# TinyMPC/tinympc-matlab

Measured on AMD Instinct MI355X. Metric: ADMM iterations/s, batched quadrotor nx=12 nu=4 N=50 (instance-iterations/s, whole job), higher is better.
Workload: dtype f64

## Files before the change

### __graft_entry__.py

```python
from __future__ import annotations

import hashlib
import importlib.util
import os
import shutil
import subprocess
import sys

ROOT = os.path.dirname(os.path.abspath(__file__))
if ROOT not in sys.path:
    sys.path.insert(0, ROOT)
PKG_DIR = os.path.join(ROOT, "tinympc-matlab_amd")
PKG_NAME = "tinympc_matlab_amd"
CSRC = os.path.join(PKG_DIR, "csrc")
HIP_LIB = os.path.join(PKG_DIR, "libtinympc_hip.so")
ORACLE_DIR = os.path.join(ROOT, "oracle")
REFERENCE_SRC = "/root/reference/src/codegen_src"

HIP_SOURCES = ["tinympc_kernels.hip", "tinympc_precompute_rows.hip", "tinympc_solve.hip", "tinympc_solve_b.hip", "tinympc_solve_fam.hip", "tinympc_solve_adapt.hip", "tinympc_imod_a.hip", "tinympc_solve_c.hip", "tinympc_solve_d.hip", "tinympc_solve_dr.hip", "tinympc_lean_d.hip", "tinympc_solve_dw.hip", "tinympc_solve_dx.hip", "tinympc_jit.hip", "tinympc_solve_m.hip", "tinympc_precompute_large.hip", "tinympc_handle.hip", "tinympc_plan.hip", "tinympc_session.hip", "tinympc_capi.hip",
               "tinympc_codegen.hip"]
HIP_LINTED = ["tinympc_precompute_rows.hip", "tinympc_solve.hip", "tinympc_solve_b.hip", "tinympc_solve_fam.hip", "tinympc_solve_adapt.hip", "tinympc_imod_a.hip",
              "tinympc_solve_c.hip", "tinympc_solve_d.hip", "tinympc_solve_dr.hip", "tinympc_lean_d.hip", "tinympc_solve_dw.hip", "tinympc_solve_dx.hip"]
JIT_EMBEDDED = ["tinympc_device.h", "tinympc_sweep.h", "tinympc_fam_red.h", "tinympc_solve_d_chain.h", "tinympc_solve_dw_chain.h", "tinympc_solve_dx_chain.h",
                "tinympc_solve_e_common.h", "tinympc_solve_dwide.h", "tinympc_solve_d.hip", "tinympc_solve_dw.hip", "tinympc_solve_dx.hip", "tinympc_solve_e.hip",
                "tinympc_solve_f.hip"]
_ROCKET = ["-DTINY_JIT_NX=6", "-DTINY_JIT_NU=3", "-DTINY_JIT_N=100", "-DTINY_JIT_CT=0", "-DTINY_JIT_FAM=1"]
_ROCKET_FAM = ["-DTINY_JIT_E_NROUND=1", "-DTINY_JIT_E_NCONE=2", "-DTINY_JIT_E_CONES={0,0,2},{0,6,8}", "-DTINY_JIT_E_NLX=1", "-DTINY_JIT_E_NLU=0"]
HIP_BUILTINS = [
    ("k_builtin_e_rocket100", "tinympc_solve_e.hip",
     _ROCKET + ["-DTINY_JIT_E_WPG=8", "-DTINY_JIT_E_WPS=2", "-DTINY_JIT_E_S=13"] + _ROCKET_FAM +
     ["-DTINY_JIT_E_GC_LDS=0", "-DTINY_JIT_E_GL_LDS=0", "-DTINY_JIT_E_LX_LDS=0", "-DTINY_JIT_E_KFAM=1", "-DTINY_JIT_E_DREG=1"]),
    ("k_builtin_f_rocket100", "tinympc_solve_f.hip", _ROCKET + ["-DTINY_JIT_F_WPG=4", "-DTINY_JIT_F_S=7"] + _ROCKET_FAM + ["-DTINY_JIT_F_KFAM=1"]),
    ("k_builtin_f_rocket100_session", "tinympc_solve_f.hip", _ROCKET + ["-DTINY_JIT_F_WPG=4", "-DTINY_JIT_F_S=7"] + _ROCKET_FAM + ["-DTINY_JIT_F_KFAM=1", "-DTINY_JIT_F_SESSION=1"]),
]
_NO_FAM = ["-DTINY_JIT_E_NROUND=0", "-DTINY_JIT_E_NCONE=0", "-DTINY_JIT_E_CONES={-1,0,0}", "-DTINY_JIT_E_NLX=0", "-DTINY_JIT_E_NLU=0"]
for _name, _nx, _nu, _N, _wpg, _S in (("cartpole20", 4, 1, 20, 2, 3), ("quadrotor50", 12, 4, 50, 4, 4)):
    for _suffix, _ct, _extra in (("", 1, []), ("_var", 0, []), ("_session", 0, ["-DTINY_JIT_F_SESSION=1"])):
# ... 44 lines not shown
        f.write(digest)


def _run(cmd, **kw):
    print("+", " ".join(cmd), flush=True)
    subprocess.run(cmd, check=True, **kw)


def device_asm_path(source: str) -> str:
    return os.path.join(BUILD_DIR, os.path.splitext(source)[0] + "-hip-amdgcn-amd-amdhsa-gfx950.s")


def _compile_one(hipcc: str, source: str, headers, force: bool) -> str:
    src = os.path.join(CSRC, source)
    obj = os.path.join(BUILD_DIR, os.path.splitext(source)[0] + ".o")
    digest = _hash([src] + headers, HIP_CFLAGS)
    if force or not _up_to_date(obj, digest):
        _run([hipcc] + HIP_CFLAGS + ["-save-temps=obj", "-c", src, "-o", obj])
        _stamp(obj, digest)
    return obj


def write_embedded_sources() -> str:
    os.makedirs(BUILD_DIR, exist_ok=True)
    out = os.path.join(BUILD_DIR, "tinympc_jit_embedded.inc")
    parts = ["// generated by __graft_entry__.write_embedded_sources() from tinympc-matlab_amd/csrc -- do not edit\n"]
    for i, name in enumerate(JIT_EMBEDDED):
        with open(os.path.join(CSRC, name)) as f:
            text = f.read()
        assert ')TINYSRC"' not in text
        pieces, cur = [], ""
# ... 233 lines not shown
```

### tinympc-matlab_amd/csrc/tinympc_device.h

```cpp
#pragma once
#ifndef __HIPCC_RTC__
#include <hip/hip_runtime.h>
#endif

namespace tinympc {

__host__ __device__ inline size_t ops_doubles(int W, int KT) { return (size_t)2 * W * KT + 3 * W; }

__host__ __device__ inline size_t table_rows(int N) { return (size_t)N + 2; }

constexpr int V_PAD = 4;
__host__ __device__ inline size_t v_rows(int N) { return (size_t)N + 1 + 2 * V_PAD; }
__host__ __device__ inline size_t tables_doubles(int W, int N) { return 3 * table_rows(N) * W + W; }

#if defined(__HIPCC__) || defined(__HIPCC_RTC__)
__device__ __forceinline__ void host_store(double *p, double v) { __hip_atomic_store(p, v, __ATOMIC_RELAXED, __HIP_MEMORY_SCOPE_SYSTEM); }
#endif

struct PrecomputeParams {
    int nx, nu;
    double rho;
    const double *A, *B, *fdyn, *Qd, *Rd;
    double *Kinf, *Pinf, *Quu_inv, *AmBKt, *APf, *BPf;
    int *info;
// ... 266 lines not shown
hipError_t launch_build_operators(const OperatorParams &p, hipStream_t stream);
hipError_t launch_build_tables(const TableParams &p, hipStream_t stream);
hipError_t launch_store_inst_refs(const InstRefStoreParams &p, hipStream_t stream);
hipError_t launch_build_inst_tables(const InstTableParams &p, hipStream_t stream);
hipError_t launch_fill_inst_models(const InstModelFillParams &p, hipStream_t stream);
hipError_t launch_store_inst_diag(const InstDiagParams &p, hipStream_t stream);
enum class SolveExt { Box, Families, Adaptive, InstRefs, InstBounds, InstModels };
hipError_t launch_solve_a(const SolveParams &p, SolveExt ext, int W, int KT, size_t lds_bytes, hipStream_t stream);
hipError_t launch_solve_b(const SolveParams &p, int W, int KT, size_t lds_bytes, hipStream_t stream);
size_t solve_b_lds_bytes(int nx, int nu, int N, int W);
constexpr int WAVES_PER_GROUP_B = 4;
bool solve_d_supported(int nx, int nu, int N, bool const_tables);
hipError_t launch_solve_d(const SolveParams &p, hipStream_t stream);
hipError_t launch_solve_d_refill(const SolveParams &p, hipStream_t stream);
hipError_t launch_solve_d_lean(const SolveParams &p, hipStream_t stream);
int solve_d_workgroups(int nu, int N, bool const_tables, int groups);
size_t solve_d_lds_bytes(int nu, int N, bool const_tables);
int solve_d_resident_workgroups(int wpg);
int solve_d_wavefronts_per_workgroup(int nu, int N, bool const_tables);
bool solve_dw_supported(int nx, int nu, int N, bool const_tables);
hipError_t launch_solve_dw(const SolveParams &p, hipStream_t stream);
int solve_dw_workgroups(int nu, int N, int groups);
size_t solve_dw_lds_bytes(int nu, int N);
bool solve_dx_supported(int nx, int nu, int N, bool const_tables);
hipError_t launch_solve_dx(const SolveParams &p, hipStream_t stream);
int solve_dx_workgroups(int nu, int N, int groups);
size_t solve_dx_lds_bytes(int nu, int N);
hipError_t launch_solve_c(const SolveParams &p, int W, int KT, size_t lds_bytes, hipStream_t stream);
hipError_t launch_build_chunk_tables(const ChunkTableParams &p, hipStream_t stream);
size_t f_input_table_doubles(int nu, int S);
// ... 50 lines not shown
```

### tinympc-matlab_amd/csrc/tinympc_plan.hip

```cpp
#include <cstring>
#include "tinympc_handle.h"

using namespace tinympc;
using namespace tinympc::host;

namespace {

void arm_completion_flag(tinympc_solver *s, SolveParams &p) {
    if (!p.host_sol) return;
    s->session_seq += 1;
    p.host_seq = (double)s->session_seq;
    s->flag_pending = true;
}

void decide_layout_d_variants(tinympc_solver *s) {
    if (!s->layout_d) return;
    if (s->d_varying < 0 && !s->tables_const()) {
        if (s->W == 16 && !s->d_jit && solve_d_supported(s->nx, s->nu, s->N, false)) {
            s->d_varying = 1;
        } else {
            s->d_varying_jit = solve_jit_supported(s->W, s->nx, s->nu, s->N, false);
            s->d_varying = s->d_varying_jit ? 1 : 0;
        }
    }
// ... 215 lines not shown
    return !jit || solve_jit_refill_supported(s->W, s->nx, s->nu, s->N, ct);
}

static bool lean_applies(const tinympc_solver *s, const LaunchPlan &pl) {
    if (pl.kernel != KernelId::D_COMPILED || s->W != 16 || pl.adaptive || pl.families || s->zero_copy_tick || s->st.max_iter <= 0)
        return false;
    if (pl.inst_models) return false;
    if (refill_applies(s, pl)) return false;
    const char *env = getenv("TINYMPC_LEAN");
    const int mode = env ? atoi(env) : -1;
    if (mode == 0) return false;
    if (mode == 1) return true;
    const bool reachable = s->st.abs_pri_tol > 0.0 && s->st.abs_dua_tol > 0.0;
    return s->st.check_termination != 1 || !reachable;
}

int launch(tinympc_solver *s, bool timed) {
    int rc;
    s->flag_pending = false;
    if ((rc = resolve_plan(s))) return rc;
    const LaunchPlan pl = current_plan(s);
    const bool fam = pl.families, adaptive = pl.adaptive;
    if (s->inst_tables() && !pl.inst_refs) {
        const bool r = s->inst.refs(), b = s->inst.bounds, m = s->inst.models;
        const char *what[3], *back[3];
        int n = 0;
        if (r) { what[n] = "per-instance references (set_x_ref_batch / set_u_ref_batch)"; back[n++] = "tinympc_set_x_ref / tinympc_set_u_ref return to shared references"; }
        if (b) { what[n] = "per-instance bounds (set_bound_constraints_batch)"; back[n++] = "tinympc_set_bound_constraints returns to shared bounds"; }
        if (m) { what[n] = "per-instance models (set_model_batch)"; back[n++] = "tinympc_clear_model_batch returns to the shared model"; }
        std::string subj, way;
// ... 88 lines not shown
    if (refill_applies(s, pl) && !p.x0_mirror && !p.u0_host && !p.host_sol) {
        if (!s->drefill && (rc = dalloc(s, &s->drefill, 1))) return rc;
        HIP_TRY(hipMemsetAsync(s->drefill, 0, sizeof(int), s->stream));
        p.refill_next = s->drefill;
    }
    if (timed) HIP_TRY(hipEventRecord(s->ev0, s->stream));
    switch (pl.kernel) {
        case KernelId::M:
            p.ctab = s->dctab;
            HIP_TRY(launch_solve_m(p, s->stream));
            break;
        case KernelId::D_JIT:
            HIP_TRY(launch_solve_jit(p, s->W, s->stream, pl.inst_models));
            break;
        case KernelId::D_COMPILED:
            if (lean_applies(s, pl) && !p.x0_mirror && !p.u0_host && !p.refill_next) HIP_TRY(launch_solve_d_lean(p, s->stream));
            else HIP_TRY(s->W == 64 ? launch_solve_dx(p, s->stream) : s->W == 32 ? launch_solve_dw(p, s->stream) : launch_solve_d(p, s->stream));
            break;
        case KernelId::E:
            p.ctab = s->dctab_e; p.chunk_len = s->e_chunk_len; p.chunk_count = s->e_wpg; p.chunk_levels = 1;
            HIP_TRY(launch_solve_e(p, s->fs, s->stream));
            break;
        case KernelId::F:
            p.ctab = s->dctab_f; p.ftab = s->dftab; p.chunk_len = s->f_chunk_len; p.chunk_count = s->f_chunks; p.chunk_levels = 4;
            arm_completion_flag(s, p);
            HIP_TRY(launch_solve_f(p, s->f_fs, s->stream));
            break;
        case KernelId::C:
            p.ctab = s->dctab; p.chunk_len = s->chunk_len; p.chunk_count = s->chunk_count; p.chunk_levels = s->chunk_levels;
            arm_completion_flag(s, p);
            HIP_TRY(launch_solve_c(p, s->W, s->KT, s->lds_bytes_c, s->stream));
// ... 57 lines not shown
    if (pl.inst_refs) {
        const std::string w = std::string(s->inst.refs() ? " per-instance-refs" : "") + (s->inst.bounds ? " per-instance-bounds" : "") +
                              (pl.inst_models ? " per-instance-models" : "");
        const char *words = w.c_str();
        if (pl.kernel == KernelId::D_JIT) {
            if ((rc = bind_device(s))) return rc;
            solve_jit_describe(s->W, s->nx, s->nu, s->N, true, false, false, buf, (size_t)len, true, pl.inst_models);
            strncat(buf, words, (size_t)len - strlen(buf) - 1);
            strncat(buf, " goal", (size_t)len - strlen(buf) - 1);
        } else if (pl.inst_models && models_want_d(s) && s->inst.d_models == 0) {
            if ((rc = bind_device(s))) return rc;
            solve_jit_describe(s->W, s->nx, s->nu, s->N, true, false, false, buf, (size_t)len, false, true);
            strncat(buf, words, (size_t)len - strlen(buf) - 1);
        } else {
            snprintf(buf, (size_t)len, "compiled-in layout=%c%s%s%s", pl.layout, words, pl.kernel == KernelId::D_COMPILED ? " goal" : "",
                     lean_applies(s, pl) ? " lean" : "");
        }
        return TINYMPC_OK;
    }
    if (!pl.adaptive && !s->f_sig.empty() && !s->f_ok && pl.kernel != KernelId::E && pl.kernel != KernelId::D_JIT && pl.kernel != KernelId::D_COMPILED)
        solve_f_describe(s->nx, s->nu, s->N, ct, pl.families, s->f_fs, buf, (size_t)len);
    else if (!pl.adaptive && !s->e_sig.empty() && !s->e_ok && pl.kernel != KernelId::F && pl.kernel != KernelId::D_JIT && pl.kernel != KernelId::D_COMPILED)
        solve_e_describe(s->nx, s->nu, s->N, ct, pl.families, s->fs, buf, (size_t)len);
    else if (pl.kernel == KernelId::F) solve_f_describe(s->nx, s->nu, s->N, ct, pl.families, s->f_fs, buf, (size_t)len);
    else if (pl.kernel == KernelId::E) solve_e_describe(s->nx, s->nu, s->N, ct, pl.families, s->fs, buf, (size_t)len);
    else if (pl.kernel == KernelId::D_JIT || (s->d_jit_asked && !s->layout_d && !s->layout_m)) {
        if ((rc = bind_device(s))) return rc;
        solve_jit_describe(s->W, s->nx, s->nu, s->N, ct, pl.families && !pl.adaptive, pl.adaptive && !pl.families, buf, (size_t)len);
        if (pl.kernel == KernelId::D_JIT && refill_applies(s, pl)) strncat(buf, " slot-refill", (size_t)len - strlen(buf) - 1);
    } else snprintf(buf, (size_t)len, "compiled-in layout=%c%s%s", pl.layout, refill_applies(s, pl) ? " slot-refill" : "", lean_applies(s, pl) ? " lean" : "");
    return TINYMPC_OK;
}

}
```

### tinympc-matlab_amd/csrc/tinympc_solve_d.hip

```cpp
#if defined(TINY_BUILTIN) && !defined(TINY_JIT)
#define TINY_JIT 1
#endif
#ifndef TINY_JIT
#include <atomic>
#endif
#include <type_traits>

#include "tinympc_device.h"
#include "tinympc_sweep.h"

#ifndef TINY_REFILL
#if defined(TINY_JIT_REFILL) && TINY_JIT_REFILL
#define TINY_REFILL 1
#else
#define TINY_REFILL 0
#endif
#endif

#ifndef TINY_LEAN
#define TINY_LEAN 0
#endif
#if TINY_LEAN && (TINY_REFILL || defined(TINY_JIT))
#error "TINY_LEAN: compiled-in plain kernels only"
#endif

#define TINY_STR2(x) #x
#define TINY_STR(x) TINY_STR2(x)
namespace tinympc {
template <int NX, int NU>
struct DStep;
}

#ifdef TINY_JIT
#define D_NX TINY_JIT_NX
#define D_NU TINY_JIT_NU
#include "tinympc_solve_d_chain.h"
#else
#define D_NX 12
// ... 3 lines not shown
#define D_NU 1
#include "tinympc_solve_d_chain.h"
#endif

namespace tinympc {

template <int I, int E, class F>
__device__ __forceinline__ void static_for(F &&f) {
    if constexpr (I < E) {
        f(std::integral_constant<int, I>{});
        static_for<I + 1, E>(f);
    }
}

constexpr int D_OPS_DOUBLES = 2 * 16 * 16;
#ifdef TINY_D_GROUP
constexpr int D_GROUP = TINY_D_GROUP;
constexpr int D_FIRST = TINY_D_FIRST;
#else
#if TINY_REFILL
constexpr int D_GROUP = 12;
constexpr int D_FIRST = 4;
#else
constexpr int D_GROUP = 23;
constexpr int D_FIRST = 4;
#endif
#endif
#ifdef TINY_JIT_VREG
constexpr int D_VREG_MAX = TINY_JIT_VREG;
#else
constexpr int D_VREG_MAX = 24;
#endif
constexpr int D_LDS_PER_CU = 160 * 1024;
__host__ __device__ constexpr int d_d_doubles(int nu, int N) { return ((N - 1) * 4 * nu + 1) & ~1; }
__host__ __device__ constexpr int d_tab_doubles(int N) { return 3 * (N + 2) * 16 + 16; }
constexpr int D_FAM_DOUBLES = 3 * MAX_LIN_ROWS * 16;
constexpr int D_ADAPT_DOUBLES = 5 * 16 * 16;
constexpr int D_IMOD_STRIDE = D_OPS_DOUBLES + 16;
constexpr int D_IMOD_WAVE_DOUBLES = 4 * D_IMOD_STRIDE;
__host__ __device__ constexpr int d_vl(int nu, int N, bool ct, int wpg, int cu_waves = 8, bool fam = false, bool adapt = false, bool imod = false) {
    const int ns = N - 1;
    const int wg_doubles = D_LDS_PER_CU / 8 * wpg / cu_waves - (imod ? 0 : D_OPS_DOUBLES) - (ct ? 0 : d_tab_doubles(N)) - (fam ? D_FAM_DOUBLES : 0) - (adapt ? D_ADAPT_DOUBLES : 0);
    const int wave_doubles = wg_doubles / wpg - d_d_doubles(nu, N) - (imod ? D_IMOD_WAVE_DOUBLES : 0);
    if (wave_doubles < 0) return -1;
    const int vlmax = wave_doubles / 64;
    const int want = ns > D_VREG_MAX ? ns - D_VREG_MAX : 0;
    return want <= vlmax ? want : -1;
}
__host__ __device__ constexpr size_t d_lds_bytes(int nu, int N, bool ct, int wpg, int vl, bool fam = false, bool adapt = false, bool imod = false) {
    return sizeof(double) * ((size_t)(imod ? 0 : D_OPS_DOUBLES) + (ct ? 0 : d_tab_doubles(N)) + (fam ? D_FAM_DOUBLES : 0) + (adapt ? D_ADAPT_DOUBLES : 0) +
                             (size_t)wpg * (vl * 64 + d_d_doubles(nu, N) + (imod ? D_IMOD_WAVE_DOUBLES : 0)));
}

__device__ __forceinline__ unsigned lds_addr(const double *p) { return lds_address(p); }
template <int OFF>
__device__ __forceinline__ double lds_read_async(unsigned addr) {
    return lds_read_issued_here<OFF>(addr);
}
template <int OFF>
__device__ __forceinline__ void lds_write_async(unsigned addr, double v) {
    static_assert(OFF >= 0 && OFF < 65536, "ds offset field is 16 bits");
    asm volatile("ds_write_b64 %0, %1 offset:%2" ::"v"(addr), "v"(v), "n"(OFF) : "memory");
}
template <int OFF>
__device__ __forceinline__ void lds_write_masked(unsigned addr, double v, unsigned long long mask) {
// ... 64 lines not shown
#ifdef TINY_CLOCK_STAMP
    const unsigned long long ck_entry = __builtin_amdgcn_s_memrealtime();
#endif
    const int lane = threadIdx.x & 63;
    const int wv = __builtin_amdgcn_readfirstlane((int)(threadIdx.x >> 6));
    const int j = lane >> 4, r = lane & 15;
    const long grp = (long)blockIdx.x * WPG + wv;
    const bool grp_ok = grp < p.groups;
    const long inst = grp * IPW + j;
    const bool is_x = r < NX;
    const bool is_u = (r >= NX) && (r < NXU);
    const bool inst_ok = grp_ok && inst < p.batch;
    const int koff = is_x ? 1 : 0;

    double *sOps = smem;
    double *sT = smem + (IMOD ? 0 : D_OPS_DOUBLES);
    double *sLin = sT + (CT ? 0 : d_tab_doubles(N));
    double *sAd = sLin + (FAM ? D_FAM_DOUBLES : 0);
    double *sV = sAd + (ADAPT ? D_ADAPT_DOUBLES : 0) + (size_t)wv * (VL * 64 + d_d_doubles(NU, N) + (IMOD ? D_IMOD_WAVE_DOUBLES : 0));
    double *sD = sV + VL * 64;
    double *sOpsW = sD + d_d_doubles(NU, N);

    if constexpr (IMOD) {
        if (grp_ok) {
            for (int i = lane; i < IPW * D_OPS_DOUBLES; i += 64) {
                const int jj = i >> 9, e = i & 511, which = e >> 8, k = (e >> 4) & 15, rr = e & 15;
                const long ib = grp * IPW + jj;
                const double *const ops_i = p.ops + (size_t)(ib < p.batch ? ib : 0) * ops_doubles(W, KT);
                const double v = (k < KT) ? ops_i[(size_t)which * W * KT + (size_t)rr * KT + k] : 0.0;
                sOpsW[jj * D_IMOD_STRIDE + e] = (FOLD && which == 1 && k >= NX) ? -p.rho * v : v;
            }
        }
    } else {
        for (int i = threadIdx.x; i < D_OPS_DOUBLES; i += 64 * WPG) {
            const int which = i >> 8, k = (i >> 4) & 15, rr = i & 15;
            const double v = (k < KT) ? p.ops[(size_t)which * W * KT + (size_t)rr * KT + k] : 0.0;
            sOps[i] = (FOLD && which == 1 && k >= NX) ? -p.rho * v : v;
        }
    }
    if constexpr (!CT)
        for (int i = threadIdx.x; i < d_tab_doubles(N); i += 64 * WPG) sT[i] = p.tables[i];
    if constexpr (ADAPT) {
        for (int i = threadIdx.x; i < D_ADAPT_DOUBLES; i += 64 * WPG) {
            const int which = i >> 8, k = (i >> 4) & 15, rr = i & 15;
            const int tbl = which == 0 ? 3 : which == 1 ? 4 : which - 2;
            sAd[i] = (k < KT) ? p.adapt[(size_t)tbl * W * KT + (size_t)rr * KT + k] : 0.0;
        }
    }
    if constexpr (FAM) {
        const double *lin_rows = p.fam + 4 * W + (size_t)3 * W * KT;
        for (int i = threadIdx.x; i < D_FAM_DOUBLES; i += 64 * WPG) {
            const int k3 = i / W, rr = i % W;
            const double v = lin_rows[1 + (size_t)k3 * W + rr];
            sLin[i] = (k3 % 3 == 2) ? 1.0 / v : v;
// ... 145 lines not shown
    double rhom = is_x ? nrho : 0.0;
#if TINY_REFILL
    double x0v = (inst_ok && is_x) ? p.x0[inst * NX + r] : 0.0;
#else
    const double x0v = (inst_ok && is_x) ? p.x0[inst * NX + r] : 0.0;
#endif
    if constexpr (HOSTX) {
        if (p.x0_mirror && inst_ok && is_x) p.x0_mirror[inst * NX + r] = x0v;
    }
    const int dIdx = j * NU + (is_u ? r - NX : 0);
    const double *const sDr = sD + dIdx;
    double *const sDw = sD + dIdx;
    const double *const sTl = sT + koff * W + r;
    const double *const sMf = (IMOD ? sOpsW + j * D_IMOD_STRIDE : sOps) + r, *const sMb = sMf + 256;
    const unsigned aV = lds_addr(sVl), aD = lds_addr(sDr), aT = lds_addr(sTl);
    const int ct = p.check_termination;
    double c0 = 0.0;
    if constexpr (K0) {
        c0 = cf;
        static_for<0, NX>([&](auto K) { c0 = fma(__shfl(x0v, (lane & 48) + K.value), sMf[K.value * 16], c0); });
    }
    double lrmc_f = 0.0;
    if constexpr (FOLD) {
        double mb[16];
        static_for<0, 16>([&](auto K) { mb[K.value] = (K.value >= NX && K.value < NXU) ? p.ops[(size_t)W * KT + (size_t)r * KT + K.value] : 0.0; });
        if constexpr (IMOD) static_for<NX, NXU>([&](auto K) { mb[K.value] = p.ops[opsI + (size_t)W * KT + (size_t)r * KT + K.value]; });
        lrmc_f = Step::acc_inputs(is_x ? lr_c + cb : cb, lr_c, mb);
    }

    bool active = inst_ok;
// ... 19 lines not shown
        else return sVl[decltype(S)::value * 64];
    };

#ifdef TINY_CLOCK_STAMP
    const unsigned long long ck_t0 = __builtin_amdgcn_s_memtime(), ck_r0 = __builtin_amdgcn_s_memrealtime();
#endif
#ifdef TINY_D_PAD
    asm volatile(".rept " TINY_STR(TINY_D_PAD) "\n\ts_nop 0\n\t.endr" ::: "memory");
#endif
#ifdef TINY_D_LOOP_ALIGN
    asm volatile(".p2align " TINY_STR(TINY_D_LOOP_ALIGN) ::: "memory");
#endif
    const int max_iter = p.max_iter;
#if TINY_LEAN
    auto iteration = [&](auto LEAN_, const int it) __attribute__((always_inline)) -> bool {
        constexpr bool LEANI = decltype(LEAN_)::value;
#else
    for (int it = 0; max_iter > 0; ++it) {
#endif
        const int it0 = __builtin_amdgcn_readfirstlane(it);
#if TINY_LEAN
        const bool final_round = !LEANI && it0 >= max_iter;
#elif TINY_REFILL
        const bool final_round = REFILL ? false : it0 >= max_iter;
#else
        const bool final_round = it0 >= max_iter;
#endif
        if constexpr (TWO_PER_SIMD) fair_share_priority<NS>(it0, simd_slot);
#if TINY_REFILL
        const bool fin = REFILL ? it_done >= max_iter : final_round;
        const bool wb = pending || (fin && active);
#else
        const bool wb = pending || (final_round && active);
#endif
        if (TINY_RARE(__ballot(wb) != 0ull)) {
            int lane_o = lane;
            asm volatile("" : "+v"(lane_o));
            const int r_o = lane_o & 15, j_o = lane_o >> 4;
            const bool x_o = r_o < NX;
#if TINY_REFILL
            int cur_o = cur;
            if constexpr (REFILL) asm volatile("" : "+v"(cur_o));
            const size_t grp_w = REFILL ? (size_t)(cur_o >> 2) : (size_t)grp;
            const int lane_w = REFILL ? (cur_o & 3) * 16 + r_o : lane_o;
#endif
            if (wb && r_o < NXU) {
// ... 99 lines not shown
                        static_for<0, NS>([&](auto S) { G[S.value] = nG[(S.value + koff) * 64]; });
                        static_for<0, NVR>([&](auto S) { Vr[S.value] = nV[(VL + S.value + koff) * 64]; });
                        static_for<0, VL>([&](auto S) { sVl[S.value * 64] = nV[(S.value + koff) * 64]; });
                        G0 = nG[0];
                        V0 = nV[0];
                        if (!x_o && r_o < NXU) {
                            const double *const nD = p.D + grp_n * (NS * DS) + (nxt & 3) * NU + (r_o - NX);
                            for (int i = 0; i < NS; ++i) sDw[i * DS] = nD[i * DS];
                        }
                    }
#endif
                }
            }
            pending = false;
        }
#if TINY_LEAN
        if (final_round || __ballot(active) == 0ull) return true;
#else
        if (final_round || __ballot(active) == 0ull) break;
#endif
        const int it1 = it0 + 1;
#if TINY_LEAN
        const bool check = !LEANI && __builtin_amdgcn_readfirstlane((int)((ct > 0) && ((it1 % ct) == 0))) != 0;
#elif TINY_REFILL
        bool chk = true, check_r = false;
        if constexpr (REFILL) {
            chk = active && (ct > 0) && (((it_done + 1) % ct) == 0);
            check_r = __ballot(chk) != 0ull;
        }
#define TINY_CHECK_PLAIN (__builtin_amdgcn_readfirstlane((int)((ct > 0) && ((it1 % ct) == 0))) != 0)
        const bool check = REFILL ? check_r : TINY_CHECK_PLAIN;
// ... 5 lines not shown
        double pri = 0.0, dua = 0.0;
        bool may = check;
        double m[16];
        load_ops(sMf, m);
        const bool adapt = ADAPT && __builtin_amdgcn_readfirstlane((int)((it0 > 0) && (it0 % 5 == 0))) != 0;
        double a_pr = 0.0, a_pn = 0.0, a_dr = 0.0, a_dn = 0.0;
        double gprev = 0.0;
        double mtr[16];
        if constexpr (ADAPT) {
            if (adapt) static_for<0, 16>([&](auto K) { mtr[K.value] = K.value < NXU ? sAd[2 * 256 + K.value * 16 + r] : 0.0; });
        }
        {
            const double lo0 = CT ? lo_c : sT[W + r], hi0 = CT ? hi_c : sT[TOFF + W + r];
            const double s = x0v + G0;
            const double snew = fmin(hi0, fmax(lo0, s));
            G0 = s - snew;
            pri = is_x ? fabs(x0v - snew) : 0.0;
            dua = is_x ? fabs(V0 - snew) : 0.0;
            if (may && !adapt) {
                const bool bad = !((pri < p.abs_pri_tol) && (dua * rho < p.abs_dua_tol));
#if TINY_REFILL
                may = __builtin_amdgcn_readfirstlane((int)wave_may_converge_d(__ballot(bad), __ballot(REFILL ? chk : active))) != 0;
#else
                may = __builtin_amdgcn_readfirstlane((int)wave_may_converge_d(__ballot(bad), __ballot(active))) != 0;
#endif
            }
#if TINY_REFILL
            if (TINY_RARE(may) && is_x && active) gV1u[REFILL ? row_offset(cur) : (unsigned)lane] = V0;
#else
            if (TINY_RARE(may) && is_x && active) gV1u[(unsigned)lane] = V0;
#endif
// ... 8 lines not shown
            }
        }
        double xcur = x0v;
        double dcur = lds_read_async<0>(aD), vcur = 0.0;
#if TINY_LEAN
        if constexpr (VL > 0 && !LEANI) vcur = lds_read_async<0>(aV);
#else
        if constexpr (VL > 0) vcur = lds_read_async<0>(aV);
#endif
        double locur = lo_c, hicur = hi_c;
        if constexpr (!CT) {
            locur = lds_read_async<W * 8>(aT);
            hicur = lds_read_async<(TOFF + W) * 8>(aT);
        }
        lds_wait_ops(m);
        auto fstep = [&](auto S) {
            constexpr int q = decltype(S)::value;
            double dn = 0.0, vn = 0.0, lon = lo_c, hin = hi_c;
            if constexpr (q + 1 < NS) dn = lds_read_async<(q + 1) * DS * 8>(aD);
#if TINY_LEAN
            if constexpr (q + 1 < VL && !LEANI) vn = lds_read_async<(q + 1) * 512>(aV);
#else
            if constexpr (q + 1 < VL) vn = lds_read_async<(q + 1) * 512>(aV);
#endif
            if constexpr (!CT && q + 1 < NS) {
                lon = lds_read_async<(q + 2) * W * 8>(aT);
                hin = lds_read_async<(TOFF + (q + 2) * W) * 8>(aT);
            }
            const double xprev = xcur;
            double snew_q;
#if TINY_LEAN
            if constexpr (LEANI) {
                if constexpr (q >= VL) {
                    if constexpr (K0 && q == 0) xcur = Step::fwd_reg0_nores(dcur, m, c0, locur, hicur, G[q], Vr[q - VL]);
                    else xcur = Step::fwd_reg_nores(xcur, dcur, m, cf, locur, hicur, G[q], Vr[q - VL]);
                    snew_q = Vr[q - VL];
                } else {
                    double vnew;
                    if constexpr (K0 && q == 0) xcur = Step::fwd_lds0_nores(dcur, m, c0, locur, hicur, G[q], vnew);
                    else xcur = Step::fwd_lds_nores(xcur, dcur, m, cf, locur, hicur, G[q], vnew);
                    lds_write_async<q * 512>(aV, vnew);
                    snew_q = vnew;
                }
            } else
#endif
            if constexpr (q >= VL) {
                if constexpr (K0 && q == 0) xcur = Step::fwd_reg0(dcur, m, c0, locur, hicur, G[q], Vr[q - VL], pri, dua);
                else xcur = Step::fwd_reg(xcur, dcur, m, cf, locur, hicur, G[q], Vr[q - VL], pri, dua);
                snew_q = Vr[q - VL];
            } else {
                double vnew;
                if constexpr (K0 && q == 0) xcur = Step::fwd_lds0(dcur, m, c0, locur, hicur, G[q], vcur, vnew, pri, dua);
                else xcur = Step::fwd_lds(xcur, dcur, m, cf, locur, hicur, G[q], vcur, vnew, pri, dua);
                lds_write_async<q * 512>(aV, vnew);
                snew_q = vnew;
// ... 10 lines not shown
                    a_pn = fmax(fmax(a_pn, fabs(snew_q)), is_x ? 0.0 : fabs(out));
                    gprev = gnew;
                }
            }
            if constexpr (FAM) {
                double gcn, gln;
                const double l = families(xcur, GCr[q], GLr[q], gcn, gln);
                if (row_ok) {
                    GCr[q] = gcn;
                    GLr[q] = gln;
                    LX[q] = l;
                }
            }
            dcur = dn;
            vcur = vn;
            if constexpr (!CT) {
                locur = lon;
                hicur = hin;
            }
        };
        constexpr int DF = D_FIRST < NS ? D_FIRST : NS;
        constexpr int NG = 1 + (NS - DF + D_GROUP - 1) / D_GROUP;
        static_for<0, NG>([&](auto Gi) {
            constexpr int s0 = Gi.value == 0 ? 0 : DF + (Gi.value - 1) * D_GROUP;
            constexpr int s1 = Gi.value == 0 ? DF : ((s0 + D_GROUP < NS) ? s0 + D_GROUP : NS);
            if (TINY_RARE(may)) {
                if constexpr (s0 > 0) {
                    if (!adapt) {
                        const bool bad = !((pri < p.abs_pri_tol) && (dua * rho < p.abs_dua_tol));
#if TINY_REFILL
// ... 8 lines not shown
                    unsigned vo = REFILL ? row_offset(cur) + (unsigned)(koff * 64) : voff;
#else
                    unsigned vo = voff;
#endif
                    double *base = gV1u;
                    asm volatile("" : "+v"(vo), "+s"(base));
                    if (active) static_for<s0, s1>([&](auto S) { (base + S.value * 64)[vo] = vget(S); });
                }
            }
            static_for<s0, s1>([&](auto S) { fstep(S); });
        });
#if TINY_REFILL
        if constexpr (REFILL) {
            if (active) it_done += 1;
        } else {
            if (active) it_done = it1;
        }
#else
        if (active) it_done = it1;
#endif

        const double nrho_lin = nrho, rhom_lin = rhom, pnref_lin = pnref;
        if constexpr (ADAPT) {
            if (adapt) {
                const double x_last = xcur, g_last = gprev;
                double pr[16];
                const double delta = rho - rho0;
                static_for<0, 16>([&](auto K) {
                    constexpr int o = K.value * 16;
                    pr[K.value] = K.value < NXU ? fma(delta, sAd[4 * 256 + o + r], sAd[3 * 256 + o + r]) : 0.0;
// ... 82 lines not shown
                        "v_add_f64 %[t], %[v2], -%[g2]\n\t"
                        "v_fma_f64 %[acc], %[rhom], %[t], %[lrmc]\n\t"
                        "v_fma_f64 %[rn], %[nrho], %[t], %[lr]"
                        : [t] "=&v"(t), [px] "=&v"(px), [acc] "=&v"(acc), [rn] "=&v"(rnext)
                        : [v1] "v"(v1), [g1] "v"(G[NS - 1]), [v2] "v"(v2), [g2] "v"(G[NS - 2]), [nrho] "s"(nrho), [lrT] "v"(lrT),
                          [rhom] "v"(rhom), [lrmc] "v"(lrmc2), [lr] "v"(lr2));
                }
                rcur = px;
            }
            auto vreq = [&](auto S) -> double {
                if constexpr (decltype(S)::value >= VL) return Vr[decltype(S)::value - VL];
                else return lds_read_async<decltype(S)::value * 512>(aV);
            };
            double v2cur = vreq(std::integral_constant<int, (NS >= 3 ? NS - 3 : 0)>{});
            lds_wait_ops(m);
            static_for<0, NS - 1>([&](auto I) {
                constexpr int s = NS - 1 - I.value;
                constexpr int s2 = s >= 2 ? s - 2 : 0;
                constexpr int s3 = s >= 3 ? s - 3 : 0;
                double v2n = 0.0;
                if constexpr (s >= 2) v2n = vreq(std::integral_constant<int, s3>{});
                const double lr2 = lr_of(std::integral_constant<int, s2>{});
                const double lrmc2 = is_x ? lr2 + cb : cb;
                double a = acc, an, rn;
                if constexpr (ADAPT) Step::bwd_v(a, px, rcur, m, v2cur, G[s2], rhom_lin, lrmc2, nrho_lin, lr2, an, rn);
                else if constexpr (FOLD) Step::bwd_fold(a, px, rcur, m, v2cur, G[s2], rhom, lrmc_f, an, rn);
                else Step::bwd(a, px, rcur, m, v2cur, G[s2], rhom, lrmc2, nrho, lr2, an, rn);
                lds_write_masked<s * DS * 8>(aD, a, wr_d);
                px = a;
                rcur = rnext;
// ... 5 lines not shown
                double a = acc;
                Step::bwd_last(a, px, rcur, m);
                lds_write_masked<0>(aD, a, wr_d);
            }
        }
#if TINY_LEAN
        return false;
    };
    const bool reachable = p.abs_pri_tol > 0.0 && p.abs_dua_tol > 0.0;
    const int last_check = ct > 0 ? (max_iter / ct) * ct : 0;
    for (int it = 0; max_iter > 0;) {
        int nres = max_iter + 1;
        if (ct > 0 && reachable) nres = (it / ct + 1) * ct;
        else if (last_check > it) nres = last_check;
        const int lean_end = __builtin_amdgcn_readfirstlane(nres - 1 < max_iter ? nres - 1 : max_iter);
        bool over = false;
        for (; it < lean_end; ++it) {
            if (iteration(std::true_type{}, it)) {
                over = true;
                break;
            }
        }
        if (over || iteration(std::false_type{}, it)) break;
        ++it;
    }
#else
    }
#endif
    lds_wait();
#ifdef TINY_CLOCK_STAMP
    const unsigned long long ck_t1 = __builtin_amdgcn_s_memtime(), ck_r1 = __builtin_amdgcn_s_memrealtime();
#endif

#if TINY_REFILL
    if constexpr (REFILL) return;
#endif
    if (inst_ok && status == 1 && r < NXU) {
        __builtin_amdgcn_fence(__ATOMIC_RELEASE, "wavefront");
// ... 22 lines not shown
#endif
    if (inst_ok && r == 0) {
        if constexpr (ADAPT) p.rho_inst[inst] = rho;
        p.istats[inst * 2 + 0] = it_done;
        p.istats[inst * 2 + 1] = status;
        if (res_valid) {
            p.dstats[inst * 4 + 0] = res_px;
            p.dstats[inst * 4 + 1] = res_dx;
            p.dstats[inst * 4 + 2] = res_pu;
            p.dstats[inst * 4 + 3] = res_du;
        }
    }
}

#if TINY_LEAN
template <int NX, int NU, int N, bool CT, int WPG, int VL>
__global__ void __launch_bounds__(64 * WPG) __attribute__((amdgpu_waves_per_eu(2, 2))) k_admm_solve_d_lean(const SolveParams p) {
    extern __shared__ __attribute__((aligned(16))) double smem[];
    k_admm_solve_d_body<NX, NU, N, CT, WPG, VL>(p, smem);
}
template <int NX, int NU, int N, int WPG, int VL>
__global__ void __launch_bounds__(64 * WPG) __attribute__((amdgpu_waves_per_eu(2, 2))) k_admm_solve_d_gbnd_lean(const SolveParams p) {
    extern __shared__ __attribute__((aligned(16))) double smem[];
    k_admm_solve_d_body<NX, NU, N, true, WPG, VL, false, false, true, false, false, true>(p, smem);
}

__host__ __device__ constexpr int d_wpg(int nu, int N, bool ct) { return d_vl(nu, N, ct, 4) >= 0 ? 4 : 8; }

template <int NX, int NU, int N, bool CT>
static hipError_t launch_d_one(const SolveParams &p, hipStream_t stream) {
// ... 238 lines not shown
```

### tinympc-matlab_amd/csrc/tinympc_solve_d_chain.h

```cpp
#if !defined(D_NX) || !defined(D_NU)
#error "define D_NX and D_NU before including tinympc_solve_d_chain.h"
#endif
#if D_NX < 1 || D_NU < 1 || D_NX + D_NU > 16
#error "layout D: 1 <= nx, 1 <= nu, nx + nu <= 16"
#endif

#ifdef TINY_CHAIN_NOALIGN
#define D_AL ""
#define D_MOV64 "v_mov_b64"
#else
#define D_AL ".p2align 3\n\t"
#ifdef TINY_CHAIN_MOV32
#define D_MOV64 "v_mov_b64"
#else
#define D_MOV64 "v_mov_b64_e64"
#endif
#endif
#if (defined(TINY_JIT) && !defined(TINY_BUILTIN)) || defined(TINY_CHAIN_NOP)
#define D_HAZ "s_nop 1\n\t" D_AL
#else
#define D_HAZ D_AL
#endif
#define D_FM_(src, i) "v_fmac_f64_dpp %[a], " src ", %[m" #i "] row_newbcast:" #i " row_mask:0xf bank_mask:0xf\n\t"
#if 0 < D_NX
// ... 266 lines not shown
    static __device__ __forceinline__ double fwd_reg_nores(double x, double d, const double (&m)[16], double cf, double lo, double hi, double &g,
                                                           double &v) {
        double a, s;
        asm volatile("v_mov_b64 %[a], %[cf]\n\t" D_HAZ D_CHAIN D_PROJECT_NORES
                     : [a] "=&v"(a), [s] "=&v"(s), [g] "+v"(g), [sn] "+v"(v)
                     : [x] "v"(x), [d] "v"(d), [cf] "v"(cf), [lo] "v"(lo), [hi] "v"(hi), D_MOPS);
        lds_reads_landed();
        return a;
    }
    static __device__ __forceinline__ double fwd_lds_nores(double x, double d, const double (&m)[16], double cf, double lo, double hi, double &g,
                                                           double &vnew) {
        double a, s;
        asm volatile(D_MOV64 " %[a], %[cf]\n\t" D_HAZ D_CHAIN D_PROJECT_NORES
                     : [a] "=&v"(a), [s] "=&v"(s), [g] "+v"(g), [sn] "=&v"(vnew)
                     : [x] "v"(x), [d] "v"(d), [cf] "v"(cf), [lo] "v"(lo), [hi] "v"(hi), D_MOPS);
        lds_reads_landed();
        return a;
    }
    static __device__ __forceinline__ double fwd_reg0_nores(double d, const double (&m)[16], double c0, double lo, double hi, double &g, double &v) {
        double a, s;
        asm volatile("v_mov_b64 %[a], %[cf]\n\t" D_HAZ D_CHAIN_IN D_PROJECT_NORES
                     : [a] "=&v"(a), [s] "=&v"(s), [g] "+v"(g), [sn] "+v"(v)
                     : [d] "v"(d), [cf] "v"(c0), [lo] "v"(lo), [hi] "v"(hi), D_MOPS);
        lds_reads_landed();
        return a;
    }
    static __device__ __forceinline__ double fwd_lds0_nores(double d, const double (&m)[16], double c0, double lo, double hi, double &g, double &vnew) {
        double a, s;
        asm volatile(D_MOV64 " %[a], %[cf]\n\t" D_HAZ D_CHAIN_IN D_PROJECT_NORES
                     : [a] "=&v"(a), [s] "=&v"(s), [g] "+v"(g), [sn] "=&v"(vnew)
// ... 136 lines not shown
```

Baseline: 1.137 billion.

## Add lean kernel variant with LDS-staged accumulator starts and hoisted termination control

Adds a new lean solve variant, on by default through an environment switch, that keeps a small table of accumulator start values in LDS. The forward step reads the next start asynchronously instead of copying a register constant into the accumulator each step. It also moves termination and writeback bookkeeping out of the inner lean iterations: a control-only first iteration runs, then unchecked lean iterations, and the slack-residual subtraction is deferred to the backward pass. This is meant to shorten the serial per-step dependency chain and the per-iteration control overhead, at the cost of extra LDS per workgroup and a more complex iteration schedule. The build hash now also tracks included .hip sources.

```diff
diff --git a/__graft_entry__.py b/__graft_entry__.py
--- a/__graft_entry__.py
+++ b/__graft_entry__.py
@@ -3,6 +3,7 @@
 import hashlib
 import importlib.util
 import os
+import re
 import shutil
 import subprocess
 import sys
@@ -17,10 +18,10 @@
 ORACLE_DIR = os.path.join(ROOT, "oracle")
 REFERENCE_SRC = "/root/reference/src/codegen_src"
 
-HIP_SOURCES = ["tinympc_kernels.hip", "tinympc_precompute_rows.hip", "tinympc_solve.hip", "tinympc_solve_b.hip", "tinympc_solve_fam.hip", "tinympc_solve_adapt.hip", "tinympc_imod_a.hip", "tinympc_solve_c.hip", "tinympc_solve_d.hip", "tinympc_solve_dr.hip", "tinympc_lean_d.hip", "tinympc_solve_dw.hip", "tinympc_solve_dx.hip", "tinympc_jit.hip", "tinympc_solve_m.hip", "tinympc_precompute_large.hip", "tinympc_handle.hip", "tinympc_plan.hip", "tinympc_session.hip", "tinympc_capi.hip",
+HIP_SOURCES = ["tinympc_kernels.hip", "tinympc_precompute_rows.hip", "tinympc_solve.hip", "tinympc_solve_b.hip", "tinympc_solve_fam.hip", "tinympc_solve_adapt.hip", "tinympc_imod_a.hip", "tinympc_solve_c.hip", "tinympc_solve_d.hip", "tinympc_solve_dr.hip", "tinympc_lean_d.hip", "tinympc_lstart_d.hip", "tinympc_solve_dw.hip", "tinympc_solve_dx.hip", "tinympc_jit.hip", "tinympc_solve_m.hip", "tinympc_precompute_large.hip", "tinympc_handle.hip", "tinympc_plan.hip", "tinympc_session.hip", "tinympc_capi.hip",
                "tinympc_codegen.hip"]
 HIP_LINTED = ["tinympc_precompute_rows.hip", "tinympc_solve.hip", "tinympc_solve_b.hip", "tinympc_solve_fam.hip", "tinympc_solve_adapt.hip", "tinympc_imod_a.hip",
-              "tinympc_solve_c.hip", "tinympc_solve_d.hip", "tinympc_solve_dr.hip", "tinympc_lean_d.hip", "tinympc_solve_dw.hip", "tinympc_solve_dx.hip"]
+              "tinympc_solve_c.hip", "tinympc_solve_d.hip", "tinympc_solve_dr.hip", "tinympc_lean_d.hip", "tinympc_lstart_d.hip", "tinympc_solve_dw.hip", "tinympc_solve_dx.hip"]
 JIT_EMBEDDED = ["tinympc_device.h", "tinympc_sweep.h", "tinympc_fam_red.h", "tinympc_solve_d_chain.h", "tinympc_solve_dw_chain.h", "tinympc_solve_dx_chain.h",
                 "tinympc_solve_e_common.h", "tinympc_solve_dwide.h", "tinympc_solve_d.hip", "tinympc_solve_dw.hip", "tinympc_solve_dx.hip", "tinympc_solve_e.hip",
                 "tinympc_solve_f.hip"]
@@ -95,7 +96,9 @@
 def _compile_one(hipcc: str, source: str, headers, force: bool) -> str:
     src = os.path.join(CSRC, source)
     obj = os.path.join(BUILD_DIR, os.path.splitext(source)[0] + ".o")
-    digest = _hash([src] + headers, HIP_CFLAGS)
+    with open(src) as f:
+        included = [os.path.join(CSRC, n) for n in re.findall(r'^#include "(\w+\.hip)"', f.read(), re.M)]
+    digest = _hash([src] + included + headers, HIP_CFLAGS)
     if force or not _up_to_date(obj, digest):
         _run([hipcc] + HIP_CFLAGS + ["-save-temps=obj", "-c", src, "-o", obj])
         _stamp(obj, digest)
diff --git a/tinympc-matlab_amd/csrc/tinympc_device.h b/tinympc-matlab_amd/csrc/tinympc_device.h
--- a/tinympc-matlab_amd/csrc/tinympc_device.h
+++ b/tinympc-matlab_amd/csrc/tinympc_device.h
@@ -304,6 +304,7 @@
 hipError_t launch_solve_d(const SolveParams &p, hipStream_t stream);
 hipError_t launch_solve_d_refill(const SolveParams &p, hipStream_t stream);
 hipError_t launch_solve_d_lean(const SolveParams &p, hipStream_t stream);
+hipError_t launch_solve_d_lean_start(const SolveParams &p, hipStream_t stream);
 int solve_d_workgroups(int nu, int N, bool const_tables, int groups);
 size_t solve_d_lds_bytes(int nu, int N, bool const_tables);
 int solve_d_resident_workgroups(int wpg);
diff --git a/tinympc-matlab_amd/csrc/tinympc_lstart_d.hip b/tinympc-matlab_amd/csrc/tinympc_lstart_d.hip
--- /dev/null
+++ b/tinympc-matlab_amd/csrc/tinympc_lstart_d.hip
@@ -0,0 +1,3 @@
+#define TINY_LEAN 1
+#define TINY_LEAN_START 1
+#include "tinympc_solve_d.hip"
diff --git a/tinympc-matlab_amd/csrc/tinympc_plan.hip b/tinympc-matlab_amd/csrc/tinympc_plan.hip
--- a/tinympc-matlab_amd/csrc/tinympc_plan.hip
+++ b/tinympc-matlab_amd/csrc/tinympc_plan.hip
@@ -253,6 +253,10 @@
     const bool reachable = s->st.abs_pri_tol > 0.0 && s->st.abs_dua_tol > 0.0;
     return s->st.check_termination != 1 || !reachable;
 }
+static bool lean_start_applies() {
+    const char *env = getenv("TINYMPC_LEAN_START");
+    return !env || atoi(env) != 0;
+}
 
 int launch(tinympc_solver *s, bool timed) {
     int rc;
@@ -371,7 +375,8 @@
             HIP_TRY(launch_solve_jit(p, s->W, s->stream, pl.inst_models));
             break;
         case KernelId::D_COMPILED:
-            if (lean_applies(s, pl) && !p.x0_mirror && !p.u0_host && !p.refill_next) HIP_TRY(launch_solve_d_lean(p, s->stream));
+            if (lean_applies(s, pl) && !p.x0_mirror && !p.u0_host && !p.refill_next)
+                HIP_TRY(lean_start_applies() ? launch_solve_d_lean_start(p, s->stream) : launch_solve_d_lean(p, s->stream));
             else HIP_TRY(s->W == 64 ? launch_solve_dx(p, s->stream) : s->W == 32 ? launch_solve_dw(p, s->stream) : launch_solve_d(p, s->stream));
             break;
         case KernelId::E:
@@ -459,7 +464,7 @@
             strncat(buf, words, (size_t)len - strlen(buf) - 1);
         } else {
             snprintf(buf, (size_t)len, "compiled-in layout=%c%s%s%s", pl.layout, words, pl.kernel == KernelId::D_COMPILED ? " goal" : "",
-                     lean_applies(s, pl) ? " lean" : "");
+                     !lean_applies(s, pl) ? "" : lean_start_applies() ? " lean lds-start" : " lean");
         }
         return TINYMPC_OK;
     }
@@ -473,8 +478,9 @@
         if ((rc = bind_device(s))) return rc;
         solve_jit_describe(s->W, s->nx, s->nu, s->N, ct, pl.families && !pl.adaptive, pl.adaptive && !pl.families, buf, (size_t)len);
         if (pl.kernel == KernelId::D_JIT && refill_applies(s, pl)) strncat(buf, " slot-refill", (size_t)len - strlen(buf) - 1);
-    } else snprintf(buf, (size_t)len, "compiled-in layout=%c%s%s", pl.layout, refill_applies(s, pl) ? " slot-refill" : "", lean_applies(s, pl) ? " lean" : "");
-    return TINYMPC_OK;
-}
-
-}
+    } else snprintf(buf, (size_t)len, "compiled-in layout=%c%s%s", pl.layout, refill_applies(s, pl) ? " slot-refill" : "",
+                  !lean_applies(s, pl) ? "" : lean_start_applies() ? " lean lds-start" : " lean");
+    return TINYMPC_OK;
+}
+
+}
diff --git a/tinympc-matlab_amd/csrc/tinympc_solve_d.hip b/tinympc-matlab_amd/csrc/tinympc_solve_d.hip
--- a/tinympc-matlab_amd/csrc/tinympc_solve_d.hip
+++ b/tinympc-matlab_amd/csrc/tinympc_solve_d.hip
@@ -22,6 +22,22 @@
 #endif
 #if TINY_LEAN && (TINY_REFILL || defined(TINY_JIT))
 #error "TINY_LEAN: compiled-in plain kernels only"
+#endif
+#ifndef TINY_LEAN_START
+#define TINY_LEAN_START 0
+#endif
+#if TINY_LEAN_START && !TINY_LEAN
+#error "TINY_LEAN_START: a variant of the lean kernels"
+#endif
+#if TINY_LEAN_START && !defined(TINY_LEAN_NO_LDS_START)
+#define TINY_LDS_START 1
+#else
+#define TINY_LDS_START 0
+#endif
+#if TINY_LEAN_START && !defined(TINY_LEAN_NO_HOIST)
+#define TINY_LEAN_HOIST 1
+#else
+#define TINY_LEAN_HOIST 0
 #endif
 
 #define TINY_STR2(x) #x
@@ -55,6 +71,7 @@
 }
 
 constexpr int D_OPS_DOUBLES = 2 * 16 * 16;
+constexpr int D_START_DOUBLES = TINY_LDS_START ? 16 : 0;
 #ifdef TINY_D_GROUP
 constexpr int D_GROUP = TINY_D_GROUP;
 constexpr int D_FIRST = TINY_D_FIRST;
@@ -81,7 +98,7 @@
 constexpr int D_IMOD_WAVE_DOUBLES = 4 * D_IMOD_STRIDE;
 __host__ __device__ constexpr int d_vl(int nu, int N, bool ct, int wpg, int cu_waves = 8, bool fam = false, bool adapt = false, bool imod = false) {
     const int ns = N - 1;
-    const int wg_doubles = D_LDS_PER_CU / 8 * wpg / cu_waves - (imod ? 0 : D_OPS_DOUBLES) - (ct ? 0 : d_tab_doubles(N)) - (fam ? D_FAM_DOUBLES : 0) - (adapt ? D_ADAPT_DOUBLES : 0);
+    const int wg_doubles = D_LDS_PER_CU / 8 * wpg / cu_waves - (imod ? 0 : D_OPS_DOUBLES + D_START_DOUBLES) - (ct ? 0 : d_tab_doubles(N)) - (fam ? D_FAM_DOUBLES : 0) - (adapt ? D_ADAPT_DOUBLES : 0);
     const int wave_doubles = wg_doubles / wpg - d_d_doubles(nu, N) - (imod ? D_IMOD_WAVE_DOUBLES : 0);
     if (wave_doubles < 0) return -1;
     const int vlmax = wave_doubles / 64;
@@ -89,7 +106,7 @@
     return want <= vlmax ? want : -1;
 }
 __host__ __device__ constexpr size_t d_lds_bytes(int nu, int N, bool ct, int wpg, int vl, bool fam = false, bool adapt = false, bool imod = false) {
-    return sizeof(double) * ((size_t)(imod ? 0 : D_OPS_DOUBLES) + (ct ? 0 : d_tab_doubles(N)) + (fam ? D_FAM_DOUBLES : 0) + (adapt ? D_ADAPT_DOUBLES : 0) +
+    return sizeof(double) * ((size_t)(imod ? 0 : D_OPS_DOUBLES + D_START_DOUBLES) + (ct ? 0 : d_tab_doubles(N)) + (fam ? D_FAM_DOUBLES : 0) + (adapt ? D_ADAPT_DOUBLES : 0) +
                              (size_t)wpg * (vl * 64 + d_d_doubles(nu, N) + (imod ? D_IMOD_WAVE_DOUBLES : 0)));
 }
 
@@ -184,7 +201,13 @@
     const int koff = is_x ? 1 : 0;
 
     double *sOps = smem;
+#if TINY_LDS_START
+    static_assert(!IMOD && !FAM && !ADAPT && !REFILL, "the table of accumulator starts: lean kernels only");
+    double *sStart = smem + D_OPS_DOUBLES;
+    double *sT = sStart + D_START_DOUBLES;
+#else
     double *sT = smem + (IMOD ? 0 : D_OPS_DOUBLES);
+#endif
     double *sLin = sT + (CT ? 0 : d_tab_doubles(N));
     double *sAd = sLin + (FAM ? D_FAM_DOUBLES : 0);
     double *sV = sAd + (ADAPT ? D_ADAPT_DOUBLES : 0) + (size_t)wv * (VL * 64 + d_d_doubles(NU, N) + (IMOD ? D_IMOD_WAVE_DOUBLES : 0));
@@ -208,6 +231,9 @@
             sOps[i] = (FOLD && which == 1 && k >= NX) ? -p.rho * v : v;
         }
     }
+#if TINY_LDS_START
+    if (threadIdx.x < D_START_DOUBLES) sStart[threadIdx.x] = p.ops[(size_t)2 * W * KT + threadIdx.x];
+#endif
     if constexpr (!CT)
         for (int i = threadIdx.x; i < d_tab_doubles(N); i += 64 * WPG) sT[i] = p.tables[i];
     if constexpr (ADAPT) {
@@ -383,6 +409,9 @@
     const double *const sTl = sT + koff * W + r;
     const double *const sMf = (IMOD ? sOpsW + j * D_IMOD_STRIDE : sOps) + r, *const sMb = sMf + 256;
     const unsigned aV = lds_addr(sVl), aD = lds_addr(sDr), aT = lds_addr(sTl);
+#if TINY_LDS_START
+    const unsigned aC = lds_addr(sStart + r);
+#endif
     const int ct = p.check_termination;
     double c0 = 0.0;
     if constexpr (K0) {
@@ -432,7 +461,11 @@
     const int max_iter = p.max_iter;
 #if TINY_LEAN
     auto iteration = [&](auto LEAN_, const int it) __attribute__((always_inline)) -> bool {
+#if TINY_LEAN_HOIST
+        constexpr bool LEANI = decltype(LEAN_)::value != 0, CTL_ONLY = decltype(LEAN_)::value == 2, NO_CTL = LEANI && !CTL_ONLY;
+#else
         constexpr bool LEANI = decltype(LEAN_)::value;
+#endif
 #else
     for (int it = 0; max_iter > 0; ++it) {
 #endif
@@ -444,10 +477,16 @@
 #else
         const bool final_round = it0 >= max_iter;
 #endif
+#if TINY_LEAN_HOIST
+        if constexpr (TWO_PER_SIMD && !CTL_ONLY) fair_share_priority<NS>(it0, simd_slot);
+#else
         if constexpr (TWO_PER_SIMD) fair_share_priority<NS>(it0, simd_slot);
+#endif
 #if TINY_REFILL
         const bool fin = REFILL ? it_done >= max_iter : final_round;
         const bool wb = pending || (fin && active);
+#elif TINY_LEAN_HOIST
+        const bool wb = NO_CTL ? false : pending || (final_round && active);
 #else
         const bool wb = pending || (final_round && active);
 #endif
@@ -577,7 +616,12 @@
             }
             pending = false;
         }
-#if TINY_LEAN
+#if TINY_LEAN_HOIST
+        if constexpr (!NO_CTL) {
+            if (final_round || __ballot(active) == 0ull) return true;
+        }
+        if constexpr (CTL_ONLY) return false;
+#elif TINY_LEAN
         if (final_round || __ballot(active) == 0ull) return true;
 #else
         if (final_round || __ballot(active) == 0ull) break;
@@ -613,7 +657,12 @@
             const double lo0 = CT ? lo_c : sT[W + r], hi0 = CT ? hi_c : sT[TOFF + W + r];
             const double s = x0v + G0;
             const double snew = fmin(hi0, fmax(lo0, s));
+#if TINY_LEAN_HOIST
+            if constexpr (LEANI) G0 = s;
+            else G0 = s - snew;
+#else
             G0 = s - snew;
+#endif
             pri = is_x ? fabs(x0v - snew) : 0.0;
             dua = is_x ? fabs(V0 - snew) : 0.0;
             if (may && !adapt) {
@@ -652,6 +701,9 @@
             hicur = lds_read_async<(TOFF + W) * 8>(aT);
         }
         lds_wait_ops(m);
+#if TINY_LDS_START
+        double acur = 0.0;
+#endif
         auto fstep = [&](auto S) {
             constexpr int q = decltype(S)::value;
             double dn = 0.0, vn = 0.0, lon = lo_c, hin = hi_c;
@@ -665,18 +717,31 @@
                 lon = lds_read_async<(q + 2) * W * 8>(aT);
                 hin = lds_read_async<(TOFF + (q + 2) * W) * 8>(aT);
             }
+#if TINY_LDS_START
+            static_assert(K0, "step 0 starts from c0");
+            double an = 0.0;
+            if constexpr (LEANI && q + 1 < NS) an = lds_read_issued_here<0>(aC);
+#endif
             const double xprev = xcur;
             double snew_q;
 #if TINY_LEAN
             if constexpr (LEANI) {
                 if constexpr (q >= VL) {
                     if constexpr (K0 && q == 0) xcur = Step::fwd_reg0_nores(dcur, m, c0, locur, hicur, G[q], Vr[q - VL]);
+#if TINY_LDS_START
+                    else xcur = Step::fwd_reg_start(xcur, dcur, m, acur, locur, hicur, G[q], Vr[q - VL]);
+#else
                     else xcur = Step::fwd_reg_nores(xcur, dcur, m, cf, locur, hicur, G[q], Vr[q - VL]);
+#endif
                     snew_q = Vr[q - VL];
                 } else {
                     double vnew;
                     if constexpr (K0 && q == 0) xcur = Step::fwd_lds0_nores(dcur, m, c0, locur, hicur, G[q], vnew);
+#if TINY_LDS_START
+                    else xcur = Step::fwd_lds_start(xcur, dcur, m, acur, locur, hicur, G[q], vnew);
+#else
                     else xcur = Step::fwd_lds_nores(xcur, dcur, m, cf, locur, hicur, G[q], vnew);
+#endif
                     lds_write_async<q * 512>(aV, vnew);
                     snew_q = vnew;
                 }
@@ -717,6 +782,9 @@
             }
             dcur = dn;
             vcur = vn;
+#if TINY_LDS_START
+            acur = an;
+#endif
             if constexpr (!CT) {
                 locur = lon;
                 hicur = hin;
@@ -755,6 +823,10 @@
         if constexpr (REFILL) {
             if (active) it_done += 1;
         } else {
+            if (active) it_done = it1;
+        }
+#elif TINY_LEAN_HOIST
+        if constexpr (!NO_CTL) {
             if (active) it_done = it1;
         }
 #else
@@ -867,6 +939,13 @@
             };
             double v2cur = vreq(std::integral_constant<int, (NS >= 3 ? NS - 3 : 0)>{});
             lds_wait_ops(m);
+#if TINY_LEAN_HOIST
+            if constexpr (LEANI) {
+                asm volatile("" : "+v"(G0));
+                G0 = G0 - V0;
+                asm volatile("" ::"v"(G0));
+            }
+#endif
             static_for<0, NS - 1>([&](auto I) {
                 constexpr int s = NS - 1 - I.value;
                 constexpr int s2 = s >= 2 ? s - 2 : 0;
@@ -902,6 +981,14 @@
         if (ct > 0 && reachable) nres = (it / ct + 1) * ct;
         else if (last_check > it) nres = last_check;
         const int lean_end = __builtin_amdgcn_readfirstlane(nres - 1 < max_iter ? nres - 1 : max_iter);
+#if TINY_LEAN_HOIST
+        if (it < lean_end) {
+            if (iteration(std::integral_constant<int, 2>{}, it)) break;
+            for (; it < lean_end; ++it) (void)iteration(std::true_type{}, it);
+            if (active) it_done = __builtin_amdgcn_readfirstlane(it);
+        }
+        if (iteration(std::false_type{}, it)) break;
+#else
         bool over = false;
         for (; it < lean_end; ++it) {
             if (iteration(std::true_type{}, it)) {
@@ -910,6 +997,7 @@
             }
         }
         if (over || iteration(std::false_type{}, it)) break;
+#endif
         ++it;
     }
 #else
@@ -962,6 +1050,12 @@
 }
 
 #if TINY_LEAN
+#if TINY_LEAN_START
+#define k_admm_solve_d_lean k_admm_solve_d_lean_start
+#define k_admm_solve_d_gbnd_lean k_admm_solve_d_gbnd_lean_start
+#define launch_solve_d_lean launch_solve_d_lean_start
+static_assert(d_vl(4, 50, true, 4) == 25, "quadrotor N=50: 25 slack slots in LDS with four wavefronts per workgroup");
+#endif
 template <int NX, int NU, int N, bool CT, int WPG, int VL>
 __global__ void __launch_bounds__(64 * WPG) __attribute__((amdgpu_waves_per_eu(2, 2))) k_admm_solve_d_lean(const SolveParams p) {
     extern __shared__ __attribute__((aligned(16))) double smem[];
diff --git a/tinympc-matlab_amd/csrc/tinympc_solve_d_chain.h b/tinympc-matlab_amd/csrc/tinympc_solve_d_chain.h
--- a/tinympc-matlab_amd/csrc/tinympc_solve_d_chain.h
+++ b/tinympc-matlab_amd/csrc/tinympc_solve_d_chain.h
@@ -304,6 +304,24 @@
         asm volatile(D_MOV64 " %[a], %[cf]\n\t" D_HAZ D_CHAIN D_PROJECT_NORES
                      : [a] "=&v"(a), [s] "=&v"(s), [g] "+v"(g), [sn] "=&v"(vnew)
                      : [x] "v"(x), [d] "v"(d), [cf] "v"(cf), [lo] "v"(lo), [hi] "v"(hi), D_MOPS);
+        lds_reads_landed();
+        return a;
+    }
+    static __device__ __forceinline__ double fwd_reg_start(double x, double d, const double (&m)[16], double a, double lo, double hi, double &g,
+                                                           double &v) {
+        double s;
+        asm volatile(D_HAZ D_CHAIN D_PROJECT_NORES
+                     : [a] "+&v"(a), [s] "=&v"(s), [g] "+v"(g), [sn] "+v"(v)
+                     : [x] "v"(x), [d] "v"(d), [lo] "v"(lo), [hi] "v"(hi), D_MOPS);
+        lds_reads_landed();
+        return a;
+    }
+    static __device__ __forceinline__ double fwd_lds_start(double x, double d, const double (&m)[16], double a, double lo, double hi, double &g,
+                                                           double &vnew) {
+        double s;
+        asm volatile(D_HAZ D_CHAIN D_PROJECT_NORES
+                     : [a] "+&v"(a), [s] "=&v"(s), [g] "+v"(g), [sn] "=&v"(vnew)
+                     : [x] "v"(x), [d] "v"(d), [lo] "v"(lo), [hi] "v"(hi), D_MOPS);
         lds_reads_landed();
         return a;
     }
```

After: 1.163 billion (median of 6 runs). 1.02x the previous value.
